# birdnet-team/birdnet-stm32

Measured on AMD Instinct MI355X. Metric: audio chunks/sec (3 s @ 24 kHz), higher is better.
Workload: dtype i8

## Files before the change

birdnet-stm32_amd/csrc/bn_i8_strip.hip:

```cpp
#include <stdlib.h>

#include "bn_kernels.h"
#include "bn_requant.h"

namespace bn {
namespace {

template <int QL> struct RawRow { int t[3][QL]; };
template <int QL> struct TRow { int c[QL][4]; };

template <int QL>
__device__ __forceinline__ RawRow<QL> load_row(__amdgpu_buffer_rsrc_t rsrc, const int voff[3], int soff) {
    RawRow<QL> r;
#pragma unroll
    for (int j = 0; j < 3; ++j) {
        if constexpr (QL == 2) {
            const v2i v = __builtin_bit_cast(v2i, __builtin_amdgcn_raw_buffer_load_b64(rsrc, voff[j], soff, 0));
            r.t[j][0] = v.x; r.t[j][1] = v.y;
        } else {
            const v4i v = __builtin_bit_cast(v4i, __builtin_amdgcn_raw_buffer_load_b128(rsrc, voff[j], soff, 0));
            r.t[j][0] = v.x; r.t[j][1] = v.y; r.t[j][2] = v.z; r.t[j][3] = v.w;
        }
    }
    return r;
// ... 223 lines not shown
                acc[t] = __builtin_amdgcn_mfma_i32_16x16x32_i8(af, bf, acc[t], 0, 0, 0);
            } else {
                const v4i af = {pwa[t][0][0], pwa[t][0][1], pwa[t][0][2], pwa[t][0][3]};
                const v4i bf = {bfrag[0], bfrag[1], bfrag[2], bfrag[3]};
                acc[t] = __builtin_amdgcn_mfma_i32_16x16x64_i8(af, bf, acc[t], 0, 0, 0);
            }
        }
    };
    auto epi_part = [&](const v4i (&acc)[NT], const int (&cenv)[QL], int oh) {
        int outw[NT];
#pragma unroll
        for (int t = 0; t < NT; ++t) {
            const v4i m = my_pw[(kq * NT + t) * 4 + 0], c1 = my_pw[(kq * NT + t) * 4 + 1], sh = my_pw[(kq * NT + t) * 4 + 2];
            const int e1 = ADD ? 0 : reinterpret_cast<const int*>(my_pw + (kq * NT + t) * 4 + 3)[0];
            const long cc[4] = {__builtin_bit_cast(long, (v2i){c1.x, c1.y}), __builtin_bit_cast(long, (v2i){c1.z, c1.w}),
                                __builtin_bit_cast(long, (v2i){sh.x, sh.y}), __builtin_bit_cast(long, (v2i){sh.z, sh.w})};
            int qv[4];
#pragma unroll
            for (int e = 0; e < 4; ++e) {
                int v = med3(ADD ? rq(acc[t][e], m[e], c1[e], sh[e]) : rq_hi(acc[t][e], m[e], cc[e], e1, e), a.pw_lo, a.pw_hi);
                if constexpr (ADD)
                    v = add_tab[(uint32_t)perm(cenv[t % QL], v, 0x0c0c0400u + (e << 8))];
                qv[e] = v;
            }
            outw[t] = perm(perm(qv[3], qv[2], 0x0c0c0400u), perm(qv[1], qv[0], 0x0c0c0400u), 0x05040100u);
        }
        const int soff = oh * a.OW * COUT;
        if constexpr (NT == 2) {
            __builtin_amdgcn_raw_buffer_store_b64(__builtin_bit_cast(__attribute__((__vector_size__(2 * sizeof(int)))) int, (v2i){outw[0], outw[1]}), rs_out, voff_out, soff, 0);
        } else {
            v4i ov = {outw[0], outw[1], outw[2], outw[3]};
            __builtin_amdgcn_raw_buffer_store_b128(__builtin_bit_cast(__attribute__((__vector_size__(4 * sizeof(int)))) int, ov), rs_out, voff_out, soff, 0);
            asm volatile("s_nop 1" : "+v"(ov));
        }
    };
    v4i pacc[NT];
    int pcen[QL] = {};
    int poh = 0;
    auto emit = [&](int i0, int i1, int i2, int oh, int step) {
        int bfrag[QL];
        dw_part(i0, i1, i2, bfrag);
        if constexpr (NW > 1 && !PIPE) {
            v2i* buf = xchg + ((step & 1) * SPB + wave / NW) * (NW * 64);
            buf[w * 64 + lane] = (v2i){bfrag[0], bfrag[1]};
            lds_barrier();
            v4i acc[NT];
            mma_part(bfrag, buf, acc);
            epi_part(acc, cen[i1], oh);
        } else if constexpr (PIPE) {
            v2i* buf = xchg + ((step & 1) * SPB + wave / NW) * (NW * 64);
            buf[w * 64 + lane] = (v2i){bfrag[0], bfrag[1]};
            if (step > 0) epi_part(pacc, pcen, poh);
            lds_barrier();
            mma_part(bfrag, buf, pacc);
#pragma unroll
            for (int ql = 0; ql < QL; ++ql) pcen[ql] = cen[i1][ql];
            poh = oh;
        } else {
            v4i acc[NT];
            mma_part(bfrag, nullptr, acc);
            epi_part(acc, cen[i1], oh);
        }
    };

    constexpr int P = 3 - S;
    issue(0, 0);
    issue(1, 1);
#pragma unroll
    for (int rr = 0; rr < P; ++rr) {
        consume(rr & 1, rr, rr % 3);
        issue(rr & 1, rr + 2);
    }
    constexpr int U = 6 / S;
    for (int k = 0; k < steps; k += U) {
#pragma unroll
        for (int u = 0; u < U; ++u) {
            if (k + u >= steps) break;
#pragma unroll
            for (int s = 0; s < S; ++s) {
                const int rs = P + S * u + s;
                consume(rs & 1, S * k + rs, rs % 3);
                issue(rs & 1, S * k + rs + 2);
            }
            emit((S * u) % 3, (S * u + 1) % 3, (S * u + 2) % 3, oh0 + k + u, k + u);
        }
    }
    if constexpr (PIPE) {
        if (steps > 0) epi_part(pacc, pcen, poh);
    }
}

__global__ __launch_bounds__(512) __attribute__((amdgpu_waves_per_eu(4))) void i8_strip_mf_kernel(Strip8Args a) {
    constexpr int CIN = 32, COUT = 32, QL = 2, NT = 2, NW = 1, SPB = 8, NTHREADS = 512;
    constexpr int nDWW = 4 * QL * 12, nDWB = 4 * QL * 4, nDWC = 4 * QL * 12, nPWA = NT * NW * 64 * QL, nPWB = 4 * NT * 4;
    constexpr int kDWW = 0, kDWB = kDWW + nDWW, kDWC = kDWB + nDWB, kPWA = kDWC + nDWC, kPWB = kPWA + nPWA, kPWC = kPWB + nPWB;
    extern __shared__ __attribute__((aligned(16))) unsigned char lds_all[];
    const unsigned char* add_tab = lds_all;
    v4i* c_dw = reinterpret_cast<v4i*>(lds_all + 65536);
    v4i* c_pw = c_dw + nDWC / 3;
    const int tid = threadIdx.x;
    {
        const v4i* src = reinterpret_cast<const v4i*>(a.cst);
        for (int i = tid; i < nDWC / 12; i += NTHREADS) {
            const v4i m = src[kDWC / 4 + 3 * i], c1 = src[kDWC / 4 + 3 * i + 1], sh = src[kDWC / 4 + 3 * i + 2];
            const long c[4] = {rq64(c1.x), rq64(c1.y), rq64(c1.z), rq64(c1.w)};
            c_dw[4 * i] = m;
            c_dw[4 * i + 1] = (v4i){(int)c[0], (int)(c[0] >> 32), (int)c[1], (int)(c[1] >> 32)};
            c_dw[4 * i + 2] = (v4i){(int)c[2], (int)(c[2] >> 32), (int)c[3], (int)(c[3] >> 32)};
            c_dw[4 * i + 3] = (v4i){pack_shifts(sh - 1), 0, 0, 0};
        }
        for (int i = tid; i < 4 * NT; i += NTHREADS) {
            c_pw[4 * i] = src[kPWC / 4 + 3 * i];
            c_pw[4 * i + 1] = src[kPWC / 4 + 3 * i + 1];
            c_pw[4 * i + 2] = src[kPWC / 4 + 3 * i + 2];
            c_pw[4 * i + 3] = (v4i){0, 0, 0, 0};
        }
        const v4i* tsrc = reinterpret_cast<const v4i*>(a.add_tab);
        v4i* tdst = reinterpret_cast<v4i*>(lds_all);
        for (int i = tid; i < 4096; i += NTHREADS) tdst[i] = tsrc[i];
    }
    __syncthreads();

    const int lane = tid & 63;
    const int wave = __builtin_amdgcn_readfirstlane(tid >> 6);
    const int n = lane & 15, g = lane >> 4;
    const int strips_x = a.OW >> 4;
    const int rblocks = (a.OH + a.TH - 1) / a.TH;
    int wid = xcd_tile(blockIdx.x, gridDim.x) * SPB + wave;
    if (wid >= a.B * strips_x * rblocks) return;
    const int sx = wid % strips_x;
    wid /= strips_x;
    const int ry = wid % rblocks;
    const int chunk = wid / rblocks;
    const int oh0 = ry * a.TH;
    const int steps = (a.OH - oh0) < a.TH ? (a.OH - oh0) : a.TH;
    const int ow = sx * 16 + n;

    v4i dwa[2][3];
    v4i dwb[2];
#pragma unroll
    for (int ct = 0; ct < 2; ++ct) {
        const int c = 16 * ct + n;
#pragma unroll
        for (int dy = 0; dy < 3; ++dy) {
            const int taps = a.cst[kDWW + (((c >> 3) * QL + ((c >> 2) & 1)) * 3 + dy) * 4 + (c & 3)];
            const int b = g < 3 ? ((taps >> (8 * g)) & 0xff) << (8 * (n & 3)) : 0;
            dwa[ct][dy] = (v4i){(n >> 2) == 0 ? b : 0, (n >> 2) == 1 ? b : 0, (n >> 2) == 2 ? b : 0, (n >> 2) == 3 ? b : 0};
        }
        dwb[ct] = reinterpret_cast<const v4i*>(a.cst + kDWB)[4 * ct + g];
    }
    long pwa[NT];
    v4i pwb[NT];
#pragma unroll
    for (int t = 0; t < NT; ++t) {
        const uint32_t lo = (uint32_t)a.cst[kPWA + (t * 64 + (n + 16 * (g >> 1))) * QL + (g & 1)];
        const uint32_t hi = (uint32_t)a.cst[kPWA + (t * 64 + (n + 16 * (2 + (g >> 1)))) * QL + (g & 1)];
        pwa[t] = (long)(((unsigned long)hi << 32) | lo);
        pwb[t] = reinterpret_cast<const v4i*>(a.cst + kPWB)[g * NT + t];
    }

    const int zp4 = (a.zp_in & 0xff) * 0x01010101;
    const v4i zrow = {zp4, zp4, zp4, zp4};
    const int icol = ow + g - 1;
    const bool outside = g < 3 && (icol < 0 || icol >= a.W);
    const bool outer = sx == 0 || sx == strips_x - 1;
    const int in_chunk_bytes = a.H * a.W * CIN, row_bytes = a.W * CIN;
    const __amdgpu_buffer_rsrc_t rs_in =
        __builtin_amdgcn_make_buffer_rsrc(const_cast<int8_t*>(a.x) + (size_t)chunk * in_chunk_bytes, 0, in_chunk_bytes, 0x00020000);
    const __amdgpu_buffer_rsrc_t rs_out =
        __builtin_amdgcn_make_buffer_rsrc(a.y + (size_t)chunk * a.OH * a.OW * COUT, 0, a.OH * a.OW * COUT, 0x00020000);
    const int ccol = g == 3 ? icol - 1 : icol;
    const int voff_b = (ccol < 0 ? 0 : (ccol >= a.W ? a.W - 1 : ccol)) * CIN;
    const int voff_r = ow * CIN + 8 * g;
    const int voff_out = ow * COUT + 8 * g;
    const int ir0 = oh0 - a.pt;
    const int rows_needed = steps + 2;

    v4i rawb[2][2];
    v2i rawr[2];
    v4i brow[3][2];
    v2i cen[3];
    auto row_ok = [&](int rr) { const int ir = ir0 + rr; return rr < rows_needed && ir >= 0 && ir < a.H; };
    auto issue = [&](int slot, int rr) {
        if (row_ok(rr)) {
            const int so = (ir0 + rr) * row_bytes;
            rawb[slot][0] = __builtin_bit_cast(v4i, __builtin_amdgcn_raw_buffer_load_b128(rs_in, voff_b, so, 0));
            rawb[slot][1] = __builtin_bit_cast(v4i, __builtin_amdgcn_raw_buffer_load_b128(rs_in, voff_b + 16, so, 0));
            rawr[slot] = __builtin_bit_cast(v2i, __builtin_amdgcn_raw_buffer_load_b64(rs_in, voff_r, so, 0));
        }
    };
    auto consume = [&](int slot, int rr, int ti) {
        if (row_ok(rr)) {
            brow[ti][0] = rawb[slot][0];
            brow[ti][1] = rawb[slot][1];
            if (outer) {
#pragma unroll
                for (int ct = 0; ct < 2; ++ct)
#pragma unroll
                    for (int e = 0; e < 4; ++e) brow[ti][ct][e] = outside ? zp4 : brow[ti][ct][e];
            }
            cen[ti] = rawr[slot];
        } else {
            brow[ti][0] = zrow;
            brow[ti][1] = zrow;
            cen[ti] = (v2i){zp4, zp4};
        }
    };
    auto emit = [&](int i0, int i1, int i2, int oh) {
        asm volatile("" ::: "memory");
        int bfrag[2];
        v4i acc[2];
#pragma unroll
        for (int ct = 0; ct < 2; ++ct) acc[ct] = __builtin_amdgcn_mfma_i32_16x16x64_i8(dwa[ct][0], brow[i0][ct], dwb[ct], 0, 0, 0);
#pragma unroll
        for (int ct = 0; ct < 2; ++ct) acc[ct] = __builtin_amdgcn_mfma_i32_16x16x64_i8(dwa[ct][1], brow[i1][ct], acc[ct], 0, 0, 0);
#pragma unroll
        for (int ct = 0; ct < 2; ++ct) acc[ct] = __builtin_amdgcn_mfma_i32_16x16x64_i8(dwa[ct][2], brow[i2][ct], acc[ct], 0, 0, 0);
#pragma unroll
        for (int ct = 0; ct < 2; ++ct) {
            const int q = 4 * ct + g;
            const v4i m = c_dw[q * 4 + 0], c01 = c_dw[q * 4 + 1], c23 = c_dw[q * 4 + 2];
            const int e1 = reinterpret_cast<const int*>(c_dw + q * 4 + 3)[0];
            const long cc[4] = {__builtin_bit_cast(long, (v2i){c01.x, c01.y}), __builtin_bit_cast(long, (v2i){c01.z, c01.w}),
                                __builtin_bit_cast(long, (v2i){c23.x, c23.y}), __builtin_bit_cast(long, (v2i){c23.z, c23.w})};
            int qv[4];
#pragma unroll
            for (int e = 0; e < 4; ++e) qv[e] = med3(rq_hi(acc[ct][e], m[e], cc[e], e1, e), a.dw_lo, a.dw_hi);
            bfrag[ct] = perm(perm(qv[3], qv[2], 0x0c0c0400u), perm(qv[1], qv[0], 0x0c0c0400u), 0x05040100u);
        }
        const long bf = ((long)(uint32_t)bfrag[1] << 32) | (uint32_t)bfrag[0];
        int outw[NT];
#pragma unroll
        for (int t = 0; t < NT; ++t) {
            const v4i pacc = __builtin_amdgcn_mfma_i32_16x16x32_i8(pwa[t], bf, pwb[t], 0, 0, 0);
            const v4i m = c_pw[(g * NT + t) * 4 + 0], c1 = c_pw[(g * NT + t) * 4 + 1], sh = c_pw[(g * NT + t) * 4 + 2];
            int qv[4];
#pragma unroll
            for (int e = 0; e < 4; ++e) {
                const int v = med3(rq(pacc[e], m[e], c1[e], sh[e]), a.pw_lo, a.pw_hi);
                qv[e] = add_tab[(uint32_t)perm(cen[i1][t], v, 0x0c0c0400u + (e << 8))];
            }
            outw[t] = perm(perm(qv[3], qv[2], 0x0c0c0400u), perm(qv[1], qv[0], 0x0c0c0400u), 0x05040100u);
        }
        __builtin_amdgcn_raw_buffer_store_b64(__builtin_bit_cast(__attribute__((__vector_size__(2 * sizeof(int)))) int, (v2i){outw[0], outw[1]}), rs_out, voff_out,
                                              oh * a.OW * COUT, 0);
    };

    issue(0, 0);
    issue(1, 1);
#pragma unroll
    for (int rr = 0; rr < 2; ++rr) {
        consume(rr & 1, rr, rr % 3);
        issue(rr & 1, rr + 2);
    }
    for (int k = 0; k < steps; k += 6) {
#pragma unroll
        for (int u = 0; u < 6; ++u) {
            if (k + u >= steps) break;
            const int rs = 2 + u;
            consume(rs & 1, k + rs, rs % 3);
            issue(rs & 1, k + rs + 2);
            emit(u % 3, (u + 1) % 3, (u + 2) % 3, oh0 + k + u);
        }
    }
}

template <int CW, int NW, int COUT, int S, bool ADD, bool W8 = false>
void launch_strip(const Strip8Args& a, hipStream_t s) {
    constexpr int SPB = ADD ? 8 / NW : (NW == 1 ? 4 : 1);
    constexpr int QL = CW / 16, NT = COUT / NW / 16;
    constexpr size_t smem = (ADD ? 65536 : 0) + (size_t)NW * (4 * QL * 16 + 4 * NT * 16) * 4 + (NW > 1 ? NW * 4 * QL * 12 * 4 + 2 * SPB * NW * 64 * 8 : 0);
    const long per_chunk = (long)(W8 ? 1 : a.OW / 16) * ((a.OH + a.TH - 1) / a.TH);
    const long blocks = NW == 1 ? (a.B * per_chunk + SPB - 1) / SPB : ((a.B + SPB - 1) / SPB) * per_chunk;
    auto kern = i8_strip_kernel<CW, NW, COUT, S, ADD, W8>;
    if (smem > 65536) (void)ensure_dynamic_lds(reinterpret_cast<const void*>(kern), smem);
    hipLaunchKernelGGL(kern, dim3((unsigned)blocks), dim3(64 * NW * SPB), smem, s, a);
}

constexpr int kF_STA = 0, kF_STB = 64, kF_STC = 80, kF_DWW = 128, kF_DWB = 176, kF_DWC = 192, kF_PWA = 240, kF_PWB = 368, kF_PWC = 400;

__global__ __launch_bounds__(256) void i8_front_strip_kernel(FrontStrip8Args a) {
    const int tid = threadIdx.x;
    const int lane = tid & 63;
    const int wave = __builtin_amdgcn_readfirstlane(tid >> 6);
    const int n = lane & 15, kq = lane >> 4;
    const int strips_x = a.OW >> 4;
    const int rblocks = (a.OH + a.TH - 1) / a.TH;
    int wid = xcd_tile(blockIdx.x, gridDim.x) * 4 + wave;
    if (wid >= a.B * strips_x * rblocks) return;
    const int sx = wid % strips_x;
    wid /= strips_x;
    const int ry = wid % rblocks;
    const int chunk = wid / rblocks;
    const int oh0 = ry * a.TH;
    const int nrows = (a.OH - oh0) < a.TH ? (a.OH - oh0) : a.TH;
    const int ow = sx * 16 + n;

    const v4i* c4 = reinterpret_cast<const v4i*>(a.cst);
    const long sta = (long)(uint32_t)a.cst[kF_STA + lane];
    const v4i stb = c4[kF_STB / 4 + kq];
    const v4i stm = c4[kF_STC / 4 + kq * 3 + 0], stc1 = c4[kF_STC / 4 + kq * 3 + 1], ste = c4[kF_STC / 4 + kq * 3 + 2];
    const long stc[4] = {rq64(stc1.x), rq64(stc1.y), rq64(stc1.z), rq64(stc1.w)};
    const int ste1 = pack_shifts(ste - 1);
    int dww[3][4];
#pragma unroll
    for (int i = 0; i < 3; ++i) {
        const v4i v = c4[kF_DWW / 4 + kq * 3 + i];
        dww[i][0] = v.x; dww[i][1] = v.y; dww[i][2] = v.z; dww[i][3] = v.w;
    }
    const v4i dwb = c4[kF_DWB / 4 + kq];
    const v4i dwm = c4[kF_DWC / 4 + kq * 3 + 0], dwc1 = c4[kF_DWC / 4 + kq * 3 + 1], dwe = c4[kF_DWC / 4 + kq * 3 + 2];
    const long dwc[4] = {rq64(dwc1.x), rq64(dwc1.y), rq64(dwc1.z), rq64(dwc1.w)};
    const int dwe1 = pack_shifts(dwe - 1);
    long pwa[2];
    v4i pwb[2], pwm[2], pwc1[2];
    int pwe1[2];
    long pwc[2][4];
#pragma unroll
    for (int t = 0; t < 2; ++t) {
        pwa[t] = (long)(uint32_t)a.cst[kF_PWA + t * 64 + lane];
        pwb[t] = c4[kF_PWB / 4 + kq * 2 + t];
        pwm[t] = c4[kF_PWC / 4 + (kq * 2 + t) * 3 + 0];
        pwc1[t] = c4[kF_PWC / 4 + (kq * 2 + t) * 3 + 1];
        pwe1[t] = pack_shifts(c4[kF_PWC / 4 + (kq * 2 + t) * 3 + 2] - 1);
#pragma unroll
        for (int e = 0; e < 4; ++e) pwc[t][e] = rq64(pwc1[t][e]);
    }

    const int zfe4 = (a.zp_fe & 0xff) * 0x01010101;
    const int zst4 = (a.zp_st & 0xff) * 0x01010101;
    const int zstrow = (a.zp_st & 0xff) * 0x00010101;
    const int fe_bytes = a.H0 * a.W0;
    const __amdgpu_buffer_rsrc_t rs_fe =
        __builtin_amdgcn_make_buffer_rsrc(const_cast<int8_t*>(a.fe) + (size_t)chunk * fe_bytes, 0, fe_bytes, 0x00020000);
    const __amdgpu_buffer_rsrc_t rs_out =
        __builtin_amdgcn_make_buffer_rsrc(a.y + (size_t)chunk * a.OH * a.OW * 32, 0, a.OH * a.OW * 32, 0x00020000);
    const bool right_fe = 4 * ow + 4 >= a.W0;
    const bool right_st = 2 * ow + 2 >= a.W0 / 2;
    const int voff_out = ow * 32 + 8 * kq;
    const int sr0 = 2 * oh0;
    const int rows_needed = 2 * (nrows - 1) + 3;

    constexpr int FD = 6;
    v2i raw[FD];
    TRow<1> T[3];

    auto fe_row = [&](int srel) { return sr0 + srel - 1 + kq; };
    auto issue = [&](int slot, int srel) {
        if (srel < rows_needed) {
            int fr = fe_row(srel);
            fr = fr < 0 ? 0 : (fr >= a.H0 ? a.H0 - 1 : fr);
            raw[slot] = __builtin_bit_cast(v2i, __builtin_amdgcn_raw_buffer_load_b64(rs_fe, fr * a.W0 + 4 * ow, 0, 0));
        }
    };
    auto stem_row = [&](int slot, int srel, int ti) {
        if (srel < rows_needed && sr0 + srel < a.H0) {
            const int fr = fe_row(srel);
            const bool ok = fr >= 0 && fr < a.H0;
            const int A = ok ? raw[slot].x : zfe4;
            const int Bd = (ok && !right_fe) ? raw[slot].y : zfe4;
            const int x[3] = {A & 0x00ffffff, perm(Bd, A, 0x0c040302u), Bd & 0x00ffffff};
            int pk[3];
#pragma unroll
            for (int j = 0; j < 3; ++j) {
                const v4i acc = __builtin_amdgcn_mfma_i32_16x16x32_i8(sta, (long)(uint32_t)x[j], stb, 0, 0, 0);
                int qv[4];
#pragma unroll
                for (int e = 0; e < 4; ++e) qv[e] = med3(rq_hi(acc[e], stm[e], stc[e], ste1, e), a.st_lo, a.st_hi);
                pk[j] = perm(perm(qv[3], qv[2], 0x0c0c0400u), perm(qv[1], qv[0], 0x0c0c0400u), 0x05040100u);
            }
            if (right_st) pk[2] = zst4;
            const int lo = perm(pk[1], pk[0], 0x05010400u);
            const int hi = perm(pk[1], pk[0], 0x07030602u);
            T[ti].c[0][0] = perm(pk[2], lo, 0x0c040100u);
            T[ti].c[0][1] = perm(pk[2], lo, 0x0c050302u);
            T[ti].c[0][2] = perm(pk[2], hi, 0x0c060100u);
            T[ti].c[0][3] = perm(pk[2], hi, 0x0c070302u);
        } else {
#pragma unroll
            for (int e = 0; e < 4; ++e) T[ti].c[0][e] = zstrow;
        }
    };
    auto emit = [&](int i0, int i1, int i2, int oh) {
        int qv[4];
#pragma unroll
        for (int e = 0; e < 4; ++e) {
            int acc = dot4_first(T[i0].c[0][e], dww[0][e], dwb[e]);
            acc = dot4(T[i1].c[0][e], dww[1][e], acc);
            acc = dot4(T[i2].c[0][e], dww[2][e], acc);
            qv[e] = med3(rq_hi(acc, dwm[e], dwc[e], dwe1, e), a.dw_lo, a.dw_hi);
        }
        const long bf = (long)(uint32_t)perm(perm(qv[3], qv[2], 0x0c0c0400u), perm(qv[1], qv[0], 0x0c0c0400u), 0x05040100u);
        int outw[2];
#pragma unroll
        for (int t = 0; t < 2; ++t) {
            const v4i acc = __builtin_amdgcn_mfma_i32_16x16x32_i8(pwa[t], bf, pwb[t], 0, 0, 0);
            int ov[4];
#pragma unroll
            for (int e = 0; e < 4; ++e) ov[e] = med3(rq_hi(acc[e], pwm[t][e], pwc[t][e], pwe1[t], e), a.pw_lo, a.pw_hi);
            outw[t] = perm(perm(ov[3], ov[2], 0x0c0c0400u), perm(ov[1], ov[0], 0x0c0c0400u), 0x05040100u);
        }
        __builtin_amdgcn_raw_buffer_store_b64(__builtin_bit_cast(__attribute__((__vector_size__(2 * sizeof(int)))) int, (v2i){outw[0], outw[1]}), rs_out, voff_out, oh * a.OW * 32, 0);
    };

#pragma unroll
    for (int rr = 0; rr < FD; ++rr) issue(rr, rr);
    stem_row(0, 0, 0);
    issue(0, FD);
    for (int k = 0; k < nrows; k += 3) {
#pragma unroll
        for (int u = 0; u < 3; ++u) {
            if (k + u >= nrows) break;
#pragma unroll
            for (int s = 0; s < 2; ++s) {
                const int rs = 1 + 2 * u + s;
                stem_row(rs % FD, 2 * k + rs, rs % 3);
                issue(rs % FD, 2 * k + rs + FD);
            }
            emit((2 * u) % 3, (2 * u + 1) % 3, (2 * u + 2) % 3, oh0 + k + u);
        }
    }
}

struct DwStream8Args {
    const int8_t* x; int8_t* y;
    const int8_t* w; const int32_t* bias; const int32_t* mult; const int32_t* shift;
    int B, H, W, C, OH, OW, TH, pt, pl, zp_in, zp_out, amin, amax, CQ, rq_right;
    int32_t* pool;
};

struct RqHi {
    long long c[4];
    int sh[4];
};
__device__ __forceinline__ void rq_hi_setup(RqHi& r, const int (&shift)[4], int zp_out) {
#pragma unroll
    for (int e = 0; e < 4; ++e) {
        const int ex = -shift[e];
        r.c[e] = (1ll << 30) + (((1ll << (ex - 1)) + (long long)zp_out * (1ll << ex)) << 31);
        r.sh[e] = ex - 1;
    }
}

#ifdef BN_TAIL_STAMPS
__device__ long long* g_dw_stamps = nullptr;
__device__ int g_dw_sel[2] = {0, 0};
constexpr int kDwStampWaves = 4096;
#define BN_DSTAMP(i) do { if (dstamp) dst_[i] = (long long)__builtin_amdgcn_s_memrealtime(); } while (0)
#else
#define BN_DSTAMP(i) do {} while (0)
#endif

template <int S, bool HI>
__global__ __launch_bounds__(256) void i8_dw_stream_kernel(DwStream8Args a) {
#ifdef BN_TAIL_STAMPS
    long long dst_[4] = {0, 0, 0, 0};
    const long dslot = ((long)blockIdx.x - (long)gridDim.x / 2) * 4 + (threadIdx.x >> 6);
    const bool dstamp = g_dw_stamps && a.C == g_dw_sel[0] && a.H == g_dw_sel[1] && dslot >= 0 && dslot < kDwStampWaves;
#endif
    BN_DSTAMP(0);
    const int tid = threadIdx.x, lane = tid & 63;
    const int wave = __builtin_amdgcn_readfirstlane(tid >> 6);
    const int CQ = a.CQ, NCOL = 64 / CQ;
    const int cq = lane % CQ, n = lane / CQ;
    const int groups = a.C / (4 * CQ);
    const int strips_x = (a.OW + NCOL - 1) / NCOL;
    const int rblocks = (a.OH + a.TH - 1) / a.TH;
    long wid = (long)xcd_tile(blockIdx.x, gridDim.x) * 4 + wave;
    if (wid >= (long)a.B * groups * strips_x * rblocks) return;
    const int g = (int)(wid % groups);
    wid /= groups;
    const int sx = (int)(wid % strips_x);
    wid /= strips_x;
    const int ry = (int)(wid % rblocks);
    const int chunk = (int)(wid / rblocks);
    const int oh0 = ry * a.TH;
    const int nrows = (a.OH - oh0) < a.TH ? (a.OH - oh0) : a.TH;
    const int ow = sx * NCOL + n;
    const bool live = ow < a.OW;
    const int c0 = 4 * (g * CQ + cq);

    int wr[3][4], bias[4], mult[4], shift[4];
    RqHi rqh;
    auto load_constants = [&]() {
        int wq[9];
#pragma unroll
        for (int t = 0; t < 9; ++t) wq[t] = *reinterpret_cast<const int*>(a.w + t * a.C + c0);
        const v4i b4 = *reinterpret_cast<const v4i*>(a.bias + c0), m4 = *reinterpret_cast<const v4i*>(a.mult + c0), s4 = *reinterpret_cast<const v4i*>(a.shift + c0);
        int sum[4] = {0, 0, 0, 0};
#pragma unroll
        for (int i = 0; i < 3; ++i) {
            const int r0 = wq[3 * i], r1 = wq[3 * i + 1], r2 = wq[3 * i + 2];
            const int lo = perm(r1, r0, 0x05010400u), hi = perm(r1, r0, 0x07030602u);
            wr[i][0] = perm(r2, lo, 0x0c040100u);
            wr[i][1] = perm(r2, lo, 0x0c050302u);
            wr[i][2] = perm(r2, hi, 0x0c060100u);
            wr[i][3] = perm(r2, hi, 0x0c070302u);
#pragma unroll
            for (int e = 0; e < 4; ++e) sum[e] = dot4(wr[i][e], 0x00010101, sum[e]);
        }
#pragma unroll
        for (int e = 0; e < 4; ++e) {
            bias[e] = b4[e] - a.zp_in * sum[e];
            mult[e] = m4[e];
            shift[e] = s4[e];
        }
        if constexpr (HI) rq_hi_setup(rqh, shift, a.zp_out);
    };
    const int zp4 = (a.zp_in & 0xff) * 0x01010101, zprow = (a.zp_in & 0xff) * 0x00010101;
    const int in_chunk_bytes = a.H * a.W * a.C;
    const int row_bytes = a.W * a.C;
    const __amdgpu_buffer_rsrc_t rs_in =
        __builtin_amdgcn_make_buffer_rsrc(const_cast<int8_t*>(a.x) + (size_t)chunk * in_chunk_bytes, 0, in_chunk_bytes, 0x00020000);
    const __amdgpu_buffer_rsrc_t rs_out =
        __builtin_amdgcn_make_buffer_rsrc(a.y + (size_t)chunk * a.OH * a.OW * a.C, 0, a.OH * a.OW * a.C, 0x00020000);
    const int iw0 = ow * S - a.pl;
    bool pad[3];
    int voff_in[3];
#pragma unroll
    for (int j = 0; j < 3; ++j) {
        pad[j] = !live || iw0 + j < 0 || iw0 + j >= a.W;
        voff_in[j] = pad[j] ? 0 : (iw0 + j) * a.C + c0;
    }
    const int voff_out = live ? ow * a.C + c0 : 0x7fff0000;
    const int ir0 = oh0 * S - a.pt;
    const int rows_needed = S * (nrows - 1) + 3;

    constexpr int D = 6;
    int raw[D][3], T[3][4];
    int psum[4] = {0, 0, 0, 0};
    auto row_ok = [&](int rr) { const int ir = ir0 + rr; return rr < rows_needed && ir >= 0 && ir < a.H; };
    auto issue = [&](int slot, int rr) {
        if (row_ok(rr)) {
            const int soff = (ir0 + rr) * row_bytes;
#pragma unroll
            for (int j = 0; j < 3; ++j) raw[slot][j] = __builtin_amdgcn_raw_buffer_load_b32(rs_in, voff_in[j], soff, 0);
        }
    };
    auto consume = [&](int slot, int rr, int ti) {
        if (row_ok(rr)) {
            const int r0 = pad[0] ? zp4 : raw[slot][0], r1 = pad[1] ? zp4 : raw[slot][1], r2 = pad[2] ? zp4 : raw[slot][2];
            const int lo = perm(r1, r0, 0x05010400u), hi = perm(r1, r0, 0x07030602u);
            T[ti][0] = perm(r2, lo, 0x0c040100u);
            T[ti][1] = perm(r2, lo, 0x0c050302u);
            T[ti][2] = perm(r2, hi, 0x0c060100u);
            T[ti][3] = perm(r2, hi, 0x0c070302u);
        } else {
#pragma unroll
            for (int e = 0; e < 4; ++e) T[ti][e] = zprow;
        }
    };
    auto emit = [&](int i0, int i1, int i2, int oh) {
        int qv[4];
#pragma unroll
        for (int e = 0; e < 4; ++e) {
            int acc = dot4_first(T[i0][e], wr[0][e], bias[e]);
            acc = dot4(T[i1][e], wr[1][e], acc);
            acc = dot4(T[i2][e], wr[2][e], acc);
            if constexpr (HI) qv[e] = med3((int)(((long long)acc * mult[e] + rqh.c[e]) >> 32) >> rqh.sh[e], a.amin, a.amax);
            else qv[e] = med3(mbqm_u(acc, mult[e], shift[e], (a.rq_right & 1) != 0) + a.zp_out, a.amin, a.amax);
            psum[e] += qv[e];
        }
        const int word = perm(perm(qv[3], qv[2], 0x0c0c0400u), perm(qv[1], qv[0], 0x0c0c0400u), 0x05040100u);
        __builtin_amdgcn_raw_buffer_store_b32(word, rs_out, voff_out, oh * a.OW * a.C, 0);
    };
    constexpr int P = 3 - S;
#pragma unroll
    for (int rr = 0; rr < D; ++rr) issue(rr, rr);
    load_constants();
#ifdef BN_TAIL_STAMPS
    asm volatile("" :: "v"(wr[0][0]), "v"(bias[3]) : "memory");
#endif
    BN_DSTAMP(1);
#pragma unroll
    for (int rr = 0; rr < P; ++rr) {
        consume(rr % D, rr, rr % 3);
        issue(rr % D, rr + D);
    }
    constexpr int U = 6 / S;
    for (int k = 0; k < nrows; k += U) {
#pragma unroll
        for (int u = 0; u < U; ++u) {
            if (k + u >= nrows) break;
#pragma unroll
            for (int s2 = 0; s2 < S; ++s2) {
                const int rs = P + S * u + s2;
                consume(rs % D, S * k + rs, rs % 3);
                issue(rs % D, S * k + rs + D);
            }
            emit((S * u) % 3, (S * u + 1) % 3, (S * u + 2) % 3, oh0 + k + u);
        }
    }
    BN_DSTAMP(2);
    if (a.pool) {
#pragma unroll
        for (int e = 0; e < 4; ++e) {
            int v = live ? psum[e] : 0;
            for (int off = CQ; off < 64; off <<= 1) v += __shfl_xor(v, off);
            if (n == 0) atomicAdd(a.pool + (size_t)chunk * a.C + c0 + e, v);
        }
    }
    BN_DSTAMP(3);
#ifdef BN_TAIL_STAMPS
    if (dstamp && lane == 0) {
        long long* o = g_dw_stamps + dslot * 6;
        for (int i = 0; i < 4; ++i) o[i] = dst_[i];
        o[4] = nrows;
        o[5] = S;
    }
#endif
}

template <int S, bool HI>
__global__ __launch_bounds__(256) void i8_stem_stream_kernel(DwStream8Args a, int SW) {
    const int tid = threadIdx.x, lane = tid & 63;
    const int wave = __builtin_amdgcn_readfirstlane(tid >> 6);
    const int CQ = a.CQ, NCOL = 64 / CQ;
    const int cq = lane % CQ, n = lane / CQ;
    const int groups = a.C / (4 * CQ);
    const int strips_x = (a.OW + NCOL - 1) / NCOL;
    const int rblocks = (a.OH + a.TH - 1) / a.TH;
    long wid = (long)xcd_tile(blockIdx.x, gridDim.x) * 4 + wave;
    if (wid >= (long)a.B * groups * strips_x * rblocks) return;
    const int g = (int)(wid % groups);
    wid /= groups;
    const int sx = (int)(wid % strips_x);
    wid /= strips_x;
    const int ry = (int)(wid % rblocks);
    const int chunk = (int)(wid / rblocks);
    const int oh0 = ry * a.TH;
    const int nrows = (a.OH - oh0) < a.TH ? (a.OH - oh0) : a.TH;
    const int ow = sx * NCOL + n;
    const bool live = ow < a.OW;
    const int c0 = 4 * (g * CQ + cq);
    int wr[3][4], bias[4], mult[4], shift[4];
#pragma unroll
    for (int e = 0; e < 4; ++e) {
        int sum = 0;
#pragma unroll
        for (int i = 0; i < 3; ++i) {
            const int k0 = a.w[(i * 3 + 0) * a.C + c0 + e], k1 = a.w[(i * 3 + 1) * a.C + c0 + e], k2 = a.w[(i * 3 + 2) * a.C + c0 + e];
            wr[i][e] = (k0 & 0xff) | ((k1 & 0xff) << 8) | ((k2 & 0xff) << 16);
            sum += k0 + k1 + k2;
        }
        bias[e] = a.bias[c0 + e] - a.zp_in * sum;
        mult[e] = a.mult[c0 + e];
        shift[e] = a.shift[c0 + e];
    }
    RqHi rqh;
    if constexpr (HI) rq_hi_setup(rqh, shift, a.zp_out);
    const int zp = a.zp_in & 0xff, zprow = zp * 0x00010101;
    const __amdgpu_buffer_rsrc_t rs_in =
        __builtin_amdgcn_make_buffer_rsrc(const_cast<int8_t*>(a.x) + (size_t)chunk * a.H * a.W, 0, a.H * a.W, 0x00020000);
    const __amdgpu_buffer_rsrc_t rs_out =
        __builtin_amdgcn_make_buffer_rsrc(a.y + (size_t)chunk * a.OH * a.OW * a.C, 0, a.OH * a.OW * a.C, 0x00020000);
    const int iw0 = ow * SW - a.pl;
    bool pad[3];
    int voff_in[3];
#pragma unroll
    for (int j = 0; j < 3; ++j) {
        pad[j] = !live || iw0 + j < 0 || iw0 + j >= a.W;
        voff_in[j] = pad[j] ? 0 : iw0 + j;
    }
    const int voff_out = live ? ow * a.C + c0 : 0x7fff0000;
    const int ir0 = oh0 * S - a.pt;
    const int rows_needed = S * (nrows - 1) + 3;
    constexpr int D = 6;
    int raw[D][3], T[3];
    auto row_ok = [&](int rr) { const int ir = ir0 + rr; return rr < rows_needed && ir >= 0 && ir < a.H; };
    auto issue = [&](int slot, int rr) {
        if (row_ok(rr)) {
            const int soff = (ir0 + rr) * a.W;
#pragma unroll
            for (int j = 0; j < 3; ++j) raw[slot][j] = __builtin_amdgcn_raw_buffer_load_b8(rs_in, voff_in[j], soff, 0);
        }
    };
    auto consume = [&](int slot, int rr, int ti) {
        if (row_ok(rr)) {
            const int b0 = pad[0] ? zp : (raw[slot][0] & 0xff), b1 = pad[1] ? zp : (raw[slot][1] & 0xff), b2 = pad[2] ? zp : (raw[slot][2] & 0xff);
            T[ti] = b0 | (b1 << 8) | (b2 << 16);
        } else {
            T[ti] = zprow;
        }
    };
    auto emit = [&](int i0, int i1, int i2, int oh) {
        int qv[4];
#pragma unroll
        for (int e = 0; e < 4; ++e) {
            int acc = dot4_first(T[i0], wr[0][e], bias[e]);
            acc = dot4(T[i1], wr[1][e], acc);
            acc = dot4(T[i2], wr[2][e], acc);
            if constexpr (HI) qv[e] = med3((int)(((long long)acc * mult[e] + rqh.c[e]) >> 32) >> rqh.sh[e], a.amin, a.amax);
            else qv[e] = med3(mbqm_u(acc, mult[e], shift[e], (a.rq_right & 1) != 0) + a.zp_out, a.amin, a.amax);
        }
        const int word = perm(perm(qv[3], qv[2], 0x0c0c0400u), perm(qv[1], qv[0], 0x0c0c0400u), 0x05040100u);
        __builtin_amdgcn_raw_buffer_store_b32(word, rs_out, voff_out, oh * a.OW * a.C, 0);
    };
    constexpr int P = 3 - S;
#pragma unroll
    for (int rr = 0; rr < D; ++rr) issue(rr, rr);
#pragma unroll
    for (int rr = 0; rr < P; ++rr) {
        consume(rr % D, rr, rr % 3);
        issue(rr % D, rr + D);
// ... 357 lines not shown
```

birdnet-stm32_amd/csrc/bn_requant.h:

```cpp
#pragma once
#include <hip/hip_runtime.h>
#include <stdint.h>

#include "bn_device.h"

namespace bn {

__device__ __forceinline__ int32_t srdhm_ref(int32_t a, int32_t b) {
    const bool overflow = (a == b) && (a == INT32_MIN);
    const int64_t ab = (int64_t)a * (int64_t)b;
    const int64_t nudge = ab >= 0 ? (1ll << 30) : (1ll - (1ll << 30));
    const int32_t r = (int32_t)((ab + nudge) / (1ll << 31));
    return overflow ? INT32_MAX : r;
}
__device__ __forceinline__ int32_t rdivpot_ref(int32_t x, int exponent) {
    const int32_t mask = (int32_t)((1u << exponent) - 1u);
    const int32_t remainder = x & mask;
    const int32_t threshold = (mask >> 1) + (x < 0 ? 1 : 0);
    return (x >> exponent) + (remainder > threshold ? 1 : 0);
}
__device__ __forceinline__ int32_t mbqm_ref(int32_t x, int32_t mult, int shift) {
    const int left = shift > 0 ? shift : 0;
    const int right = shift > 0 ? 0 : -shift;
    return rdivpot_ref(srdhm_ref(x * (1 << left), mult), right);
}

__device__ __forceinline__ int32_t srdhm_pos(int32_t x, int32_t m) {
    return (int32_t)(((int64_t)x * (int64_t)m + (1ll << 30)) >> 31);
}
__device__ __forceinline__ int32_t rdivpot_fast(int32_t v, int e) {
    const int32_t half = e ? (1 << (e - 1)) : 0;
    const int32_t adj = e ? (v >> 31) : 0;
    return (v + half + adj) >> e;
}
__device__ __forceinline__ int32_t mbqm(int32_t x, int32_t mult, int shift) {
    if (shift <= 0 && mult >= 0) return rdivpot_fast(srdhm_pos(x, mult), -shift);
    return mbqm_ref(x, mult, shift);
}

__device__ __forceinline__ int32_t mbqm_right(int32_t x, int32_t mult, int shift) {
    const int e = -shift;
    const int32_t v = srdhm_pos(x, mult);
    return (v + (1 << (e - 1)) + (v >> 31)) >> e;
}
__device__ __forceinline__ int32_t mbqm_u(int32_t x, int32_t mult, int shift, bool all_right) {
    return all_right ? mbqm_right(x, mult, shift) : mbqm(x, mult, shift);
}

__device__ __forceinline__ int32_t clampi(int32_t v, int32_t lo, int32_t hi) { return v < lo ? lo : (v > hi ? hi : v); }

__device__ __forceinline__ int med3(int v, int lo, int hi) {
    int r;
    asm("v_med3_i32 %0, %1, %2, %3" : "=v"(r) : "v"(v), "v"(lo), "v"(hi));
    return r;
}
__device__ __forceinline__ int perm(int s0, int s1, uint32_t sel) { return (int)__builtin_amdgcn_perm((uint32_t)s0, (uint32_t)s1, sel); }
__device__ __forceinline__ int dot4(int a, int b, int c) { return __builtin_amdgcn_sdot4(a, b, c, false); }
__device__ __forceinline__ int dot4_first(int a, int b, int c) {
    int r;
    asm("v_dot4_i32_i8 %0, %1, %2, %3" : "=v"(r) : "v"(a), "v"(b), "v"(c));
    return r;
}
__device__ __forceinline__ int pack4(const int (&q)[4]) {
    const uint32_t lo = __builtin_amdgcn_perm((uint32_t)q[1], (uint32_t)q[0], 0x0c0c0400u), hi = __builtin_amdgcn_perm((uint32_t)q[3], (uint32_t)q[2], 0x0c0c0400u);
    return (int)__builtin_amdgcn_perm(hi, lo, 0x05040100u);
}

__device__ __forceinline__ int rq(int x, int m, int c1, int e) {
    const int v = srdhm_pos(x, m);
    return (v + c1 + (v >> 31)) >> e;
}

__device__ __forceinline__ long rq64(int c1) { return ((long)c1 << 31) + 0x40000000L; }
__device__ __forceinline__ int pack_shifts(v4i sh) { return sh.x | (sh.y << 8) | (sh.z << 16) | (sh.w << 24); }
__device__ __forceinline__ int ashr_byte(int packed, int v, int e) {
    int r;
    switch (e) {
        case 0: asm("v_ashrrev_i32_sdwa %0, %1, %2 dst_sel:DWORD dst_unused:UNUSED_PAD src0_sel:BYTE_0 src1_sel:DWORD" : "=v"(r) : "v"(packed), "v"(v)); break;
        case 1: asm("v_ashrrev_i32_sdwa %0, %1, %2 dst_sel:DWORD dst_unused:UNUSED_PAD src0_sel:BYTE_1 src1_sel:DWORD" : "=v"(r) : "v"(packed), "v"(v)); break;
        case 2: asm("v_ashrrev_i32_sdwa %0, %1, %2 dst_sel:DWORD dst_unused:UNUSED_PAD src0_sel:BYTE_2 src1_sel:DWORD" : "=v"(r) : "v"(packed), "v"(v)); break;
        default: asm("v_ashrrev_i32_sdwa %0, %1, %2 dst_sel:DWORD dst_unused:UNUSED_PAD src0_sel:BYTE_3 src1_sel:DWORD" : "=v"(r) : "v"(packed), "v"(v)); break;
    }
    return r;
}
__device__ __forceinline__ int rq_hi(int x, int m, long c, int e1_packed, int e) {
    return ashr_byte(e1_packed, (int)(((long)x * (long)m + c) >> 32), e);
}

constexpr int32_t kMeanFloatForm = 0x7fffff00;
__device__ __forceinline__ int32_t mean_q(int32_t raw_sum, int32_t P, int32_t zp_in, int32_t mult, int32_t shift, int32_t zp_out) {
#pragma clang fp contract(off)
    if (shift == kMeanFloatForm) {
        const float scale = __int_as_float(mult);
        const float bias = (float)(-zp_in) * scale;
        const float mean = (float)raw_sum / (float)P;
        const float t = mean * scale;
        const float r = roundf(t + bias) + (float)zp_out;
        return (int32_t)fminf(fmaxf(r, -128.0f), 127.0f);
    }
    return clampi(mbqm(raw_sum - zp_in * P, mult, shift) + zp_out, -128, 127);
}

}
```

Measured before the change: 2.289 million.

## Fuse requant shift+pack via SDWA byte deposits and stage requant constants in LDS

Reworks the stem/depthwise/pointwise requantization: the clamp is moved before the per-channel shift using pre-shifted bounds, and the shift plus byte packing is done with SDWA byte-select writes instead of separate shifts and perm chains. Depthwise and pointwise requant constants are staged into LDS per wave and reloaded in the emit loop rather than held in registers, aiming to lower VGPR pressure and instruction count. Input row loads drop the clamp/branch and use a linear offset, relying on buffer bounds checking; right-edge padding is applied by masking. Risks include added LDS reads per row, inline asm constraining scheduling, and relying on out-of-bounds buffer loads returning zero.

```diff
diff --git a/birdnet-stm32_amd/csrc/bn_i8_strip.hip b/birdnet-stm32_amd/csrc/bn_i8_strip.hip
--- a/birdnet-stm32_amd/csrc/bn_i8_strip.hip
+++ b/birdnet-stm32_amd/csrc/bn_i8_strip.hip
@@ -549,6 +549,9 @@
     const v4i stm = c4[kF_STC / 4 + kq * 3 + 0], stc1 = c4[kF_STC / 4 + kq * 3 + 1], ste = c4[kF_STC / 4 + kq * 3 + 2];
     const long stc[4] = {rq64(stc1.x), rq64(stc1.y), rq64(stc1.z), rq64(stc1.w)};
     const int ste1 = pack_shifts(ste - 1);
+    int stlo[4], sthi[4];
+#pragma unroll
+    for (int e = 0; e < 4; ++e) shifted_bounds(a.st_lo, a.st_hi, ste[e] - 1, stlo[e], sthi[e]);
     int dww[3][4];
 #pragma unroll
     for (int i = 0; i < 3; ++i) {
@@ -556,26 +559,40 @@
         dww[i][0] = v.x; dww[i][1] = v.y; dww[i][2] = v.z; dww[i][3] = v.w;
     }
     const v4i dwb = c4[kF_DWB / 4 + kq];
-    const v4i dwm = c4[kF_DWC / 4 + kq * 3 + 0], dwc1 = c4[kF_DWC / 4 + kq * 3 + 1], dwe = c4[kF_DWC / 4 + kq * 3 + 2];
-    const long dwc[4] = {rq64(dwc1.x), rq64(dwc1.y), rq64(dwc1.z), rq64(dwc1.w)};
-    const int dwe1 = pack_shifts(dwe - 1);
+    __shared__ v4i cq_lds[4][4][3][5];
+    auto stage_quad = [&](v4i* q, v4i m, v4i c1, v4i sh, int lo, int hi) {
+        int blo[4], bhi[4];
+        long c[4];
+#pragma unroll
+        for (int e = 0; e < 4; ++e) {
+            c[e] = rq64(c1[e]);
+            shifted_bounds(lo, hi, sh[e] - 1, blo[e], bhi[e]);
+        }
+        if (n == 0) {
+            q[0] = m;
+            q[1] = (v4i){(int)c[0], (int)(c[0] >> 32), (int)c[1], (int)(c[1] >> 32)};
+            q[2] = (v4i){(int)c[2], (int)(c[2] >> 32), (int)c[3], (int)(c[3] >> 32)};
+            q[3] = (v4i){blo[0], blo[1], blo[2], blo[3]};
+            q[4] = (v4i){bhi[0], bhi[1], bhi[2], bhi[3]};
+        }
+        return pack_shifts(sh - 1);
+    };
+    const int dwe1 = stage_quad(cq_lds[wave][kq][0], c4[kF_DWC / 4 + kq * 3 + 0], c4[kF_DWC / 4 + kq * 3 + 1], c4[kF_DWC / 4 + kq * 3 + 2], a.dw_lo, a.dw_hi);
     long pwa[2];
-    v4i pwb[2], pwm[2], pwc1[2];
+    v4i pwb[2];
     int pwe1[2];
-    long pwc[2][4];
 #pragma unroll
     for (int t = 0; t < 2; ++t) {
         pwa[t] = (long)(uint32_t)a.cst[kF_PWA + t * 64 + lane];
         pwb[t] = c4[kF_PWB / 4 + kq * 2 + t];
-        pwm[t] = c4[kF_PWC / 4 + (kq * 2 + t) * 3 + 0];
-        pwc1[t] = c4[kF_PWC / 4 + (kq * 2 + t) * 3 + 1];
-        pwe1[t] = pack_shifts(c4[kF_PWC / 4 + (kq * 2 + t) * 3 + 2] - 1);
-#pragma unroll
-        for (int e = 0; e < 4; ++e) pwc[t][e] = rq64(pwc1[t][e]);
-    }
+        const v4i* pc = c4 + kF_PWC / 4 + (kq * 2 + t) * 3;
+        pwe1[t] = stage_quad(cq_lds[wave][kq][1 + t], pc[0], pc[1], pc[2], a.pw_lo, a.pw_hi);
+    }
+    const v4i* my_cq = cq_lds[wave][kq][0];
 
     const int zfe4 = (a.zp_fe & 0xff) * 0x01010101;
     const int zst4 = (a.zp_st & 0xff) * 0x01010101;
+    const bool last_strip = sx == strips_x - 1;
     const int zstrow = (a.zp_st & 0xff) * 0x00010101;
     const int fe_bytes = a.H0 * a.W0;
     const __amdgpu_buffer_rsrc_t rs_fe =
@@ -584,6 +601,7 @@
         __builtin_amdgcn_make_buffer_rsrc(a.y + (size_t)chunk * a.OH * a.OW * 32, 0, a.OH * a.OW * 32, 0x00020000);
     const bool right_fe = 4 * ow + 4 >= a.W0;
     const bool right_st = 2 * ow + 2 >= a.W0 / 2;
+    const int pad_st = right_st ? 0x00ff0000 : 0;
     const int voff_out = ow * 32 + 8 * kq;
     const int sr0 = 2 * oh0;
     const int rows_needed = 2 * (nrows - 1) + 3;
@@ -593,12 +611,9 @@
     TRow<1> T[3];
 
     auto fe_row = [&](int srel) { return sr0 + srel - 1 + kq; };
+    const int fe_off0 = (sr0 - 1 + kq) * a.W0 + 4 * ow;
     auto issue = [&](int slot, int srel) {
-        if (srel < rows_needed) {
-            int fr = fe_row(srel);
-            fr = fr < 0 ? 0 : (fr >= a.H0 ? a.H0 - 1 : fr);
-            raw[slot] = __builtin_bit_cast(v2i, __builtin_amdgcn_raw_buffer_load_b64(rs_fe, fr * a.W0 + 4 * ow, 0, 0));
-        }
+        raw[slot] = __builtin_bit_cast(v2i, __builtin_amdgcn_raw_buffer_load_b64(rs_fe, fe_off0 + srel * a.W0, 0, 0));
     };
     auto stem_row = [&](int slot, int srel, int ti) {
         if (srel < rows_needed && sr0 + srel < a.H0) {
@@ -607,46 +622,52 @@
             const int A = ok ? raw[slot].x : zfe4;
             const int Bd = (ok && !right_fe) ? raw[slot].y : zfe4;
             const int x[3] = {A & 0x00ffffff, perm(Bd, A, 0x0c040302u), Bd & 0x00ffffff};
-            int pk[3];
 #pragma unroll
             for (int j = 0; j < 3; ++j) {
                 const v4i acc = __builtin_amdgcn_mfma_i32_16x16x32_i8(sta, (long)(uint32_t)x[j], stb, 0, 0, 0);
-                int qv[4];
-#pragma unroll
-                for (int e = 0; e < 4; ++e) qv[e] = med3(rq_hi(acc[e], stm[e], stc[e], ste1, e), a.st_lo, a.st_hi);
-                pk[j] = perm(perm(qv[3], qv[2], 0x0c0c0400u), perm(qv[1], qv[0], 0x0c0c0400u), 0x05040100u);
-            }
-            if (right_st) pk[2] = zst4;
-            const int lo = perm(pk[1], pk[0], 0x05010400u);
-            const int hi = perm(pk[1], pk[0], 0x07030602u);
-            T[ti].c[0][0] = perm(pk[2], lo, 0x0c040100u);
-            T[ti].c[0][1] = perm(pk[2], lo, 0x0c050302u);
-            T[ti].c[0][2] = perm(pk[2], hi, 0x0c060100u);
-            T[ti].c[0][3] = perm(pk[2], hi, 0x0c070302u);
+                int h[4];
+#pragma unroll
+                for (int e = 0; e < 4; ++e) h[e] = med3(rq_h(acc[e], stm[e], stc[e]), stlo[e], sthi[e]);
+                deposit_column(T[ti].c[0], h, ste1, j);
+            }
+            if (last_strip) {
+#pragma unroll
+                for (int e = 0; e < 4; ++e) T[ti].c[0][e] = (T[ti].c[0][e] & ~pad_st) | (zst4 & pad_st);
+            }
         } else {
 #pragma unroll
             for (int e = 0; e < 4; ++e) T[ti].c[0][e] = zstrow;
         }
     };
     auto emit = [&](int i0, int i1, int i2, int oh) {
-        int qv[4];
+        asm volatile("" ::: "memory");
+        struct Quad { v4i m; long c[4]; int lo[4], hi[4]; };
+        auto quad = [&](int i) {
+            const v4i m = my_cq[5 * i], c01 = my_cq[5 * i + 1], c23 = my_cq[5 * i + 2], lo = my_cq[5 * i + 3], hi = my_cq[5 * i + 4];
+            return Quad{m, {__builtin_bit_cast(long, (v2i){c01.x, c01.y}), __builtin_bit_cast(long, (v2i){c01.z, c01.w}),
+                            __builtin_bit_cast(long, (v2i){c23.x, c23.y}), __builtin_bit_cast(long, (v2i){c23.z, c23.w})},
+                        {lo.x, lo.y, lo.z, lo.w}, {hi.x, hi.y, hi.z, hi.w}};
+        };
+        int h[4];
+        const Quad dq = quad(0);
 #pragma unroll
         for (int e = 0; e < 4; ++e) {
             int acc = dot4_first(T[i0].c[0][e], dww[0][e], dwb[e]);
             acc = dot4(T[i1].c[0][e], dww[1][e], acc);
             acc = dot4(T[i2].c[0][e], dww[2][e], acc);
-            qv[e] = med3(rq_hi(acc, dwm[e], dwc[e], dwe1, e), a.dw_lo, a.dw_hi);
-        }
-        const long bf = (long)(uint32_t)perm(perm(qv[3], qv[2], 0x0c0c0400u), perm(qv[1], qv[0], 0x0c0c0400u), 0x05040100u);
-        int outw[2];
+            h[e] = rq_h(acc, dq.m[e], dq.c[e]);
+        }
+        const long bf = (long)(uint32_t)clamp_deposit_quad(h, dq.lo, dq.hi, dwe1);
+        int ov[2][4];
 #pragma unroll
         for (int t = 0; t < 2; ++t) {
             const v4i acc = __builtin_amdgcn_mfma_i32_16x16x32_i8(pwa[t], bf, pwb[t], 0, 0, 0);
-            int ov[4];
-#pragma unroll
-            for (int e = 0; e < 4; ++e) ov[e] = med3(rq_hi(acc[e], pwm[t][e], pwc[t][e], pwe1[t], e), a.pw_lo, a.pw_hi);
-            outw[t] = perm(perm(ov[3], ov[2], 0x0c0c0400u), perm(ov[1], ov[0], 0x0c0c0400u), 0x05040100u);
-        }
+            const Quad pq = quad(1 + t);
+#pragma unroll
+            for (int e = 0; e < 4; ++e) ov[t][e] = med3(rq_h(acc[e], pq.m[e], pq.c[e]), pq.lo[e], pq.hi[e]);
+        }
+        int outw[2];
+        deposit_two_quads(outw[0], outw[1], ov[0], ov[1], pwe1[0], pwe1[1]);
         __builtin_amdgcn_raw_buffer_store_b64(__builtin_bit_cast(__attribute__((__vector_size__(2 * sizeof(int)))) int, (v2i){outw[0], outw[1]}), rs_out, voff_out, oh * a.OW * 32, 0);
     };
 
diff --git a/birdnet-stm32_amd/csrc/bn_requant.h b/birdnet-stm32_amd/csrc/bn_requant.h
--- a/birdnet-stm32_amd/csrc/bn_requant.h
+++ b/birdnet-stm32_amd/csrc/bn_requant.h
@@ -87,6 +87,57 @@
     return ashr_byte(e1_packed, (int)(((long)x * (long)m + c) >> 32), e);
 }
 
+__device__ __forceinline__ int rq_h(int x, int m, long c) { return (int)(((long)x * (long)m + c) >> 32); }
+
+__device__ __forceinline__ void shifted_bounds(int lo, int hi, int e1, int& blo, int& bhi) {
+    blo = lo << e1;
+    bhi = ((hi + 1) << e1) - 1;
+}
+#define BN_DEP(dst, src, J, E, MODE) \
+    "v_ashrrev_i32_sdwa " dst ", %[sh], " src " dst_sel:BYTE_" #J " dst_unused:UNUSED_" MODE " src0_sel:BYTE_" #E " src1_sel:DWORD\n\t"
+#define BN_DEP_COLUMN(J, MODE, CONSTRAINT, TAIL)                                                                                  \
+    asm(BN_DEP("%[t0]", "%[h0]", J, 0, MODE) BN_DEP("%[t1]", "%[h1]", J, 1, MODE) BN_DEP("%[t2]", "%[h2]", J, 2, MODE)            \
+            BN_DEP("%[t3]", "%[h3]", J, 3, MODE) TAIL                                                                             \
+        : [t0] CONSTRAINT(t[0]), [t1] CONSTRAINT(t[1]), [t2] CONSTRAINT(t[2]), [t3] CONSTRAINT(t[3])                              \
+        : [sh] "v"(sh), [h0] "v"(h[0]), [h1] "v"(h[1]), [h2] "v"(h[2]), [h3] "v"(h[3]))
+__device__ __forceinline__ void deposit_column(int (&t)[4], const int (&h)[4], int sh, int j) {
+    switch (j) {
+        case 0: BN_DEP_COLUMN(0, "PAD", "=&v", ""); break;
+        case 1: BN_DEP_COLUMN(1, "PRESERVE", "+v", ""); break;
+        default: BN_DEP_COLUMN(2, "PRESERVE", "+v", "s_nop 0"); break;
+    }
+}
+__device__ __forceinline__ int clamp_deposit_quad(int (&h)[4], const int (&lo)[4], const int (&hi)[4], int sh) {
+    int d;
+    asm("v_med3_i32 %[h0], %[h0], %[l0], %[u0]\n\t"
+        "v_med3_i32 %[h1], %[h1], %[l1], %[u1]\n\t"
+        BN_DEP("%[d]", "%[h0]", 0, 0, "PAD")
+        "v_med3_i32 %[h2], %[h2], %[l2], %[u2]\n\t"
+        BN_DEP("%[d]", "%[h1]", 1, 1, "PRESERVE")
+        "v_med3_i32 %[h3], %[h3], %[l3], %[u3]\n\t"
+        BN_DEP("%[d]", "%[h2]", 2, 2, "PRESERVE")
+        "s_nop 0\n\t"
+        BN_DEP("%[d]", "%[h3]", 3, 3, "PRESERVE")
+        "s_nop 0"
+        : [d] "=&v"(d), [h0] "+v"(h[0]), [h1] "+v"(h[1]), [h2] "+v"(h[2]), [h3] "+v"(h[3])
+        : [sh] "v"(sh), [l0] "v"(lo[0]), [l1] "v"(lo[1]), [l2] "v"(lo[2]), [l3] "v"(lo[3]), [u0] "v"(hi[0]), [u1] "v"(hi[1]), [u2] "v"(hi[2]),
+          [u3] "v"(hi[3]));
+    return d;
+}
+__device__ __forceinline__ void deposit_two_quads(int& d0, int& d1, const int (&a)[4], const int (&b)[4], int sha, int shb) {
+    asm("v_ashrrev_i32_sdwa %[d0], %[sa], %[a0] dst_sel:BYTE_0 dst_unused:UNUSED_PAD src0_sel:BYTE_0 src1_sel:DWORD\n\t"
+        "v_ashrrev_i32_sdwa %[d1], %[sb], %[b0] dst_sel:BYTE_0 dst_unused:UNUSED_PAD src0_sel:BYTE_0 src1_sel:DWORD\n\t"
+        "v_ashrrev_i32_sdwa %[d0], %[sa], %[a1] dst_sel:BYTE_1 dst_unused:UNUSED_PRESERVE src0_sel:BYTE_1 src1_sel:DWORD\n\t"
+        "v_ashrrev_i32_sdwa %[d1], %[sb], %[b1] dst_sel:BYTE_1 dst_unused:UNUSED_PRESERVE src0_sel:BYTE_1 src1_sel:DWORD\n\t"
+        "v_ashrrev_i32_sdwa %[d0], %[sa], %[a2] dst_sel:BYTE_2 dst_unused:UNUSED_PRESERVE src0_sel:BYTE_2 src1_sel:DWORD\n\t"
+        "v_ashrrev_i32_sdwa %[d1], %[sb], %[b2] dst_sel:BYTE_2 dst_unused:UNUSED_PRESERVE src0_sel:BYTE_2 src1_sel:DWORD\n\t"
+        "v_ashrrev_i32_sdwa %[d0], %[sa], %[a3] dst_sel:BYTE_3 dst_unused:UNUSED_PRESERVE src0_sel:BYTE_3 src1_sel:DWORD\n\t"
+        "v_ashrrev_i32_sdwa %[d1], %[sb], %[b3] dst_sel:BYTE_3 dst_unused:UNUSED_PRESERVE src0_sel:BYTE_3 src1_sel:DWORD"
+        : [d0] "=&v"(d0), [d1] "=&v"(d1)
+        : [sa] "v"(sha), [sb] "v"(shb), [a0] "v"(a[0]), [a1] "v"(a[1]), [a2] "v"(a[2]), [a3] "v"(a[3]), [b0] "v"(b[0]), [b1] "v"(b[1]),
+          [b2] "v"(b[2]), [b3] "v"(b[3]));
+}
+
 constexpr int32_t kMeanFloatForm = 0x7fffff00;
 __device__ __forceinline__ int32_t mean_q(int32_t raw_sum, int32_t P, int32_t zp_in, int32_t mult, int32_t shift, int32_t zp_out) {
 #pragma clang fp contract(off)
```

Measured after the change: 2.331 million (median of 6 runs). 1.8% higher.
